# guzba/zippy

Hardware: AMD Instinct MI355X
Metric: GiB/s uncompressed throughput (compress BestSpeed + uncompress), 4096x1 MiB batch (higher is better)
Workload: dtype u8

## Files before the change

### zippy_amd/csrc/zh_l1_match.hip

```cpp
#include <cstdlib>
#include <cstring>

#include "zh_common.h"
#include "zh_kprof.h"
#include "zh_tables.h"

namespace {
constexpr uint32_t kHashMul = 0x1e35a7bdu;
constexpr uint32_t kCntWords = 1024;
constexpr uint32_t kBitsWords = 512, kFlagBits = 12, kFlagWords = (1u << kFlagBits) / 32u;
static_assert(kBitsWords + 2u * kFlagWords <= kCntWords, "the parse's maps lie inside the coverage bitmap's words");
constexpr uint32_t kHistWords = ZH_HIST_STRIDE / 2;
static_assert(ZH_HIST_STRIDE % 2 == 0, "packed pairs");
struct __attribute__((packed)) Bytes16 {
  uint32_t x, y, z, w;
};

}

template <bool kLdsTable>
__global__ __launch_bounds__(64) void zh_l1_match_kernel(const uint8_t* __restrict__ d_src,
                                                         ZhCompressArgs a, int huffman_only,
                                                         uint16_t* __restrict__ table_pool,
                                                         uint32_t* __restrict__ next_frag,
                                                         const uint32_t* __restrict__ order,
                                                         uint32_t* __restrict__ cost, uint32_t ticket_base) {
  __shared__ uint32_t s_hist[kHistWords];
  __shared__ uint32_t s_scr[kCntWords];
  __shared__ uint32_t s_nmatch;
  uint32_t* const s_bits = s_scr;
  uint32_t* const s_seen = s_scr + kBitsWords;
  uint32_t* const s_dup = s_seen + kFlagWords;
  uint32_t* const s_cover = s_scr;

  const unsigned lane = zh_lane();
  __shared__ uint16_t s_table_lds[kLdsTable ? 16384 : 2];
  uint16_t* const s_table = kLdsTable ? s_table_lds : table_pool + (size_t)blockIdx.x * 16384u;
  uint32_t taken = 0;
  for (uint32_t ticket = ticket_base + blockIdx.x; ticket < a.nfrags; taken++) {
  const uint32_t f = order ? order[ticket] : ticket;
  const uint64_t t_start = zh_clock();
  KPROF_DECL(16);
  const ZhFragDesc fd = a.frags[f];
  const uint32_t n = fd.len;
  const uint8_t* src = d_src + fd.src_off;
  uint16_t* m_pos = a.m_pos + (size_t)f * ZH_MAX_MATCHES_PER_FRAG;
  uint16_t* m_len = a.m_len + (size_t)f * ZH_MAX_MATCHES_PER_FRAG;
  uint16_t* m_off = a.m_off + (size_t)f * ZH_MAX_MATCHES_PER_FRAG;

  const uint32_t mis = (uint32_t)((uintptr_t)src & 3u);
  const uint32_t* asrc = reinterpret_cast<const uint32_t*>(src - mis);
  const uint32_t last_dw = n ? (n + mis - 1u) >> 2 : 0u;
  auto dw = [&](uint32_t i) -> uint32_t { return asrc[i < last_dw ? i : last_dw]; };
  auto ld32 = [&](uint32_t p) -> uint32_t {
    const uint32_t q = p + mis, i = q >> 2;
    return __builtin_amdgcn_alignbyte(dw(i + 1), dw(i), q);
  };
  uint32_t table_size = 256, shift = 24;
  while (table_size < 16384u && table_size < n) {
    table_size <<= 1;
    shift--;
  }
  const uint32_t e0 = (!huffman_only && n >= 4) ? (((ld32(0) * kHashMul) >> 17) & 1u) << 15 : 0u;
  for (uint32_t i = lane; i < kBitsWords + 2u * kFlagWords; i += 64) s_scr[i] = 0;
  zh_wave_sync();
  KPROF_MARK(0);

  {
    uint32_t nm = 0;
    if (!huffman_only && n >= 15) {
      const uint32_t ip_limit = n - 15;
      uint32_t ip = 1;
      uint32_t K = 0;
      bool post = false;
      bool finished = false;
      while (!finished) {
        const bool dense = post || K < 32u;
        uint32_t pos, step, W0 = 0;
        if (dense) {
          W0 = post ? ip - 1u : ip;
          pos = W0 + lane;
          step = 1;
        } else {
          const uint32_t s = 32 + K, q = s >> 5, r = s & 31u, j = lane;
          uint32_t off = q * j;
          if (j > 32u - r) off += j - (32u - r);
          if (j > 64u - r) off += j - (64u - r);
          pos = ip + off;
          step = (s + j) >> 5;
        }
        const bool valid = pos + step <= ip_limit;
        if (!valid) pos = 1;
        Bytes16 av = {0, 0, 0, 0};
        if (valid) av = *reinterpret_cast<const Bytes16*>(src + pos);
        const uint32_t a0 = av.x, a1 = av.y, a2 = av.z, a3 = av.w;
        const uint32_t hp = a0 * kHashMul;
        const uint32_t h = hp >> shift, tag = (hp >> 17) & 1u;
        uint32_t oldw = e0;
        if (valid && ((s_bits[h >> 5] >> (h & 31u)) & 1u))
          oldw = kLdsTable ? (uint32_t)s_table[h]
                           : (uint32_t)__hip_atomic_load(s_table + h, __ATOMIC_RELAXED, __HIP_MEMORY_SCOPE_AGENT);
        const uint32_t old = oldw & 0x7fffu;
        const bool fetch = valid && (oldw >> 15) == tag;
        const uint32_t ck = (h & ((1u << kFlagBits) - 1u)) >> 5, cb = 1u << (h & 31u);
        const uint32_t seen_before = valid ? atomicOr(&s_seen[ck], cb) : 0u;
        Bytes16 qv = {0, 0, 0, 0};
        if (fetch) qv = *reinterpret_cast<const Bytes16*>(src + old);
        if (seen_before & cb) atomicOr(&s_dup[ck], cb);
        zh_wave_sync();
        const bool flagged = valid && (s_dup[ck] & cb);
        zh_wave_sync();
        if (valid) s_seen[ck] = s_dup[ck] = 0;
        const uint32_t x0 = fetch ? a0 ^ qv.x : 1u;
        const uint32_t x1 = a1 ^ qv.y;
        const uint32_t x2 = a2 ^ qv.z;
        const uint32_t x3 = a3 ^ qv.w;
        const uint32_t c0 = min(((uint32_t)__ffs((int)x0) - 1u) >> 3, 4u);
        const uint32_t c1 = min(((uint32_t)__ffs((int)x1) - 1u) >> 3, 4u);
        const uint32_t c2 = min(((uint32_t)__ffs((int)x2) - 1u) >> 3, 4u);
        const uint32_t c3 = min(((uint32_t)__ffs((int)x3) - 1u) >> 3, 4u);
        const uint32_t c23 = c2 + (c2 == 4u ? c3 : 0u);
        const uint32_t c123 = c1 + (c1 == 4u ? c23 : 0u);
        const uint32_t eqlen = c0 + (c0 == 4u ? c123 : 0u);

        const uint64_t V = __ballot(valid);
        const uint64_t H = __ballot(valid && x0 == 0);
        const uint64_t C = __ballot(flagged);
        uint64_t Cw = C;
        if (C && __popcll(C) <= 16) {
          Cw = 0;
          for (uint64_t cm = C; cm; cm &= cm - 1) {
            const uint32_t g = (uint32_t)__ffsll((long long)cm) - 1u;
            const uint32_t hg = __builtin_amdgcn_readlane(h, g);
            const bool same_h = valid && h == hg;
            if (__ballot(same_h) & ((1ull << g) - 1ull)) Cw |= 1ull << g;
          }
        }
        const uint32_t t = V == ~0ull ? 64u : (uint32_t)__ffsll((long long)~V) - 1u;

        KPROF_MARK(1);
        KPROF_COUNT(6, 1);
#ifndef ZH_EMU
        __builtin_amdgcn_s_setprio(1);
#endif
        uint64_t ins = post ? 1ull : 0ull;
        uint32_t i = post ? 1u : 0u;
        bool reprobe = post;
        uint32_t hop = 0x8000u;
        if (dense) {
          const uint64_t ev = (H | Cw) >> lane;
          const uint32_t d = ev ? (uint32_t)__ffsll((long long)ev) - 1u : 64u;
          const uint32_t info = eqlen | ((uint32_t)((Cw >> lane) & 1ull) << 5);
          const uint32_t gi = (uint32_t)__shfl((int)info, (int)((lane + d) & 63u), 64);
          if (d < 32u && gi < 16u) {
            const uint32_t g0 = lane + d, nx = g0 + gi;
            hop = g0 | 0x40u | (nx << 8) | ((d + 1u) << 16) | ((nx <= 64u ? nx - 1u : g0) << 22);
          } else if (!ev && lane >= 32u) {
            hop = 63u | (64u << 8);
          }
        }
        const uint32_t tt = ip_limit > W0 ? ip_limit - W0 : 0u;
        for (;;) {
          if (dense && i < 64u) {
            uint64_t sel = 0;
            uint32_t cur = zh_bcast(i), tv = 0x8000u;
            KPROF_MARK(3);
            bool go = true;
            if (!reprobe && K) {
              tv = __builtin_amdgcn_readlane(hop, cur);
              go = !(tv & 0x8000u) && (tv & 0x40u) && K + ((tv & 63u) - cur) <= 31u;
            }
            const uint32_t lim = zh_bcast(tt < 64u ? tt : 64u);
            if (go && cur < lim) {
#ifdef ZH_EMU
              do {
                tv = __builtin_amdgcn_readlane(hop, cur);
                if ((tv & 0x8040u) != 0x40u) break;
                const uint32_t g = tv & 63u, nxt = (tv >> 8) & 127u;
                sel |= 1ull << g;
                ins |= (~0ull << cur) & (~0ull >> (63u - g));
                ins |= 1ull << (nxt <= 64u ? nxt - 1u : g);
                cur = nxt;
              } while (cur < lim);
#else
              uint32_t t0, g, nxt;
              uint64_t m1;
              asm volatile(
                  "1:\n\t"
                  "v_readlane_b32 %[tv], %[hop], %[cur]\n\t"
                  "s_bitcmp1_b32 %[tv], 6\n\t"
                  "s_cbranch_scc0 2f\n\t"
                  "s_and_b32 %[g], %[tv], 63\n\t"
                  "s_bitset1_b64 %[sel], %[g]\n\t"
                  "s_bfe_u32 %[t0], %[tv], 0x60010\n\t"
                  "s_bfm_b64 %[m1], %[t0], %[cur]\n\t"
                  "s_or_b64 %[ins], %[ins], %[m1]\n\t"
                  "s_bfe_u32 %[t0], %[tv], 0x60016\n\t"
                  "s_bitset1_b64 %[ins], %[t0]\n\t"
                  "s_bfe_u32 %[cur], %[tv], 0x70008\n\t"
                  "s_cmp_lt_u32 %[cur], %[lim]\n\t"
                  "s_cbranch_scc1 1b\n\t"
                  "2:"
                  : [tv] "=&s"(tv), [cur] "+s"(cur), [sel] "+s"(sel), [ins] "+s"(ins), [t0] "=&s"(t0),
                    [g] "=&s"(g), [nxt] "=&s"(nxt), [m1] "=&s"(m1)
                  : [hop] "v"(hop), [lim] "s"(lim)
                  : "scc");
#endif
            }
            const bool chained = cur != i;
            bool run_out = false;
            if (go && cur < lim && !(tv & 0x8040u) && tt >= 64u) {
              K = (chained || reprobe ? 63u : K + 64u) - cur;
              ins |= ~0ull << cur;
              run_out = true;
            }
            KPROF_MARK(2);
            if (sel) {
              KPROF_COUNT(8, __popcll(sel));
              if ((sel >> lane) & 1ull) {
                const uint32_t k = nm + (uint32_t)__popcll(sel & zh_lanemask_lt());
                zh_store_nt(m_pos + k, (uint16_t)pos);
                zh_store_nt(m_len + k, (uint16_t)eqlen);
                zh_store_nt(m_off + k, (uint16_t)(pos - old));
              }
              nm += (uint32_t)__popcll(sel);
            }
            if (run_out) {
              post = false;
              ip = W0 + 64u;
              break;
            }
            if (chained) {
              K = 0;
              if (cur >= tt) {
                finished = true;
                break;
              }
              if (cur >= 64u) {
                post = true;
                ip = W0 + cur;
                break;
              }
              i = cur;
              reprobe = true;
            }
          }
          KPROF_COUNT(9, 1);
          if (i >= t) {
            finished = true;
            break;
          }
          uint32_t g = i;
          if (!reprobe) {
            const uint32_t last_dense = dense ? i + (31u - K) : 63u;
            uint32_t lim = last_dense < 63u ? last_dense : 63u;
            if (t - 1u < lim) lim = t - 1u;
            const uint64_t E = (H | Cw) & (~0ull << i);
            g = E ? (uint32_t)__ffsll((long long)E) - 1u : 64u;
            if (g > lim) {
              KPROF_COUNT(12, 1);
              ins |= (~0ull << i) & (~0ull >> (63u - lim));
              if (dense && lim == last_dense) {
                K = 32;
                ip = W0 + lim + 1u;
                post = false;
              } else if (lim + 1u == t && t < 64u) {
                finished = true;
              } else {
                K += 64u - i;
                post = false;
                if (dense) {
                  ip = W0 + 64u;
                } else {
                  ip = __builtin_amdgcn_readlane(pos, 63) + __builtin_amdgcn_readlane(step, 63);
                }
              }
              break;
            }
            if (g > i) ins |= (~0ull << i) & ((1ull << g) - 1ull);
            K += g - i;
          }
          uint32_t cand, flen;
          bool hit;
          if ((Cw >> g) & 1ull) {
            KPROF_COUNT(14, 1);
            const uint32_t hg = __builtin_amdgcn_readlane(h, g);
            const uint64_t same = __ballot(h == hg) & ins;
            if (same) {
              const uint32_t k = 63u - (uint32_t)__clzll((long long)same);
              cand = __builtin_amdgcn_readlane(pos, k);
              hit = __builtin_amdgcn_readlane(a0, k) == __builtin_amdgcn_readlane(a0, g);
              flen = 4;
              if (hit) {
                const uint32_t y1 = (uint32_t)__builtin_amdgcn_readlane(a1, k) ^ (uint32_t)__builtin_amdgcn_readlane(a1, g);
                if (y1) {
                  flen = 4u + (((uint32_t)__ffs((int)y1) - 1u) >> 3);
                } else {
                  const uint32_t y2 = (uint32_t)__builtin_amdgcn_readlane(a2, k) ^ (uint32_t)__builtin_amdgcn_readlane(a2, g);
                  if (y2) {
                    flen = 8u + (((uint32_t)__ffs((int)y2) - 1u) >> 3);
                  } else {
                    const uint32_t y3 = (uint32_t)__builtin_amdgcn_readlane(a3, k) ^ (uint32_t)__builtin_amdgcn_readlane(a3, g);
                    flen = y3 ? 12u + (((uint32_t)__ffs((int)y3) - 1u) >> 3) : 16u;
                  }
                }
              }
            } else {
              cand = __builtin_amdgcn_readlane(old, g);
              hit = (H >> g) & 1ull;
              flen = __builtin_amdgcn_readlane(eqlen, g);
            }
          } else {
            cand = __builtin_amdgcn_readlane(old, g);
            hit = (H >> g) & 1ull;
            flen = __builtin_amdgcn_readlane(eqlen, g);
          }
          ins |= 1ull << g;
          if (!hit) {
            if (reprobe) {
              reprobe = false;
              K = 0;
            } else {
              K++;
            }
            i = g + 1u;
            if (dense && K == 32u) {
              ip = W0 + i;
              post = false;
              break;
            }
            if (i >= 64u) {
              post = false;
              ip = dense ? W0 + 64u
                         : __builtin_amdgcn_readlane(pos, 63) + __builtin_amdgcn_readlane(step, 63);
              break;
            }
            continue;
          }
          const uint32_t mp = __builtin_amdgcn_readlane(pos, g);
          const uint32_t limit = n < mp + 258u ? n : mp + 258u;
          uint32_t matched;
          if (flen < 16u) {
            KPROF_COUNT(15, 1);
            matched = flen;
          } else {
            KPROF_COUNT(10, 1);
            zh_wave_sync();
            const uint32_t o = flen + 4u * lane;
            uint32_t avail = 0;
            if (mp + o < limit) avail = limit - (mp + o) < 4u ? limit - (mp + o) : 4u;
            const uint32_t x = ld32(mp + o) ^ ld32(cand + o);
            uint32_t eq = min(((uint32_t)__ffs((int)x) - 1u) >> 3, 4u);
            if (eq > avail) eq = avail;
            const uint64_t stop = __ballot(eq < 4u);
            const uint32_t fl = (uint32_t)__ffsll((long long)stop) - 1u;
            matched = flen + 4u * fl + __builtin_amdgcn_readlane(eq, fl);
          }
          if (matched > limit - mp) matched = limit - mp;
          if (lane == 0) {
            zh_store_nt(m_pos + nm, (uint16_t)mp);
            zh_store_nt(m_len + nm, (uint16_t)matched);
            zh_store_nt(m_off + nm, (uint16_t)(mp - cand));
          }
          nm++;
          ip = mp + matched;
          K = 0;
          post = true;
          if (ip >= ip_limit) {
            finished = true;
            break;
          }
          const uint32_t ni = g + matched;
          if (!dense || ni >= 64u) break;
          ins |= 1ull << (ni - 1u);
          i = ni;
          reprobe = true;
        }
        KPROF_MARK(3);
#ifndef ZH_EMU
        __builtin_amdgcn_s_setprio(0);
#endif
        if (finished) break;
        const bool mine = (ins >> lane) & 1ull;
        if (mine) atomicOr(&s_bits[h >> 5], 1u << (h & 31u));
        if (mine && !((C >> lane) & 1ull)) s_table[h] = (uint16_t)(pos | (tag << 15));
        uint64_t cc = ins & C;
        while (cc) {
          const uint32_t jx = (uint32_t)__ffsll((long long)cc) - 1u;
          cc &= cc - 1;
          if (lane == jx) s_table[h] = (uint16_t)(pos | (tag << 15));
        }
        zh_wave_sync();
        KPROF_MARK(4);
      }
    }
    if (lane == 0) s_nmatch = nm;
  }
  __threadfence_block();
  zh_wave_sync();
  KPROF_MARK(3);
  const uint32_t nmatch = s_nmatch;
  for (uint32_t i = lane; i < kCntWords; i += 64) s_scr[i] = 0;
  for (uint32_t i = lane; i < kHistWords; i += 64) s_hist[i] = 0;
  zh_wave_sync();

  uint32_t extra_bits = 0, covered = 0;
  auto hist_add = [&](uint32_t sym) { atomicAdd(&s_hist[sym >> 1], 1u << (16u * (sym & 1u))); };
  {
    const uint32_t mlast = nmatch ? nmatch - 1u : 0u;
    auto at = [&](uint32_t m) { return m < nmatch ? m : mlast; };
    uint32_t pq = m_pos[at(lane)], lq = m_len[at(lane)], oq = m_off[at(lane)];
    for (uint32_t m = lane; m - lane < nmatch; m += 64) {
      const uint32_t p = pq, l = lq, o = oq;
      pq = m_pos[at(m + 64u)];
      lq = m_len[at(m + 64u)];
      oq = m_off[at(m + 64u)];
      if (m < nmatch) {
        const uint32_t li = zh_len_code(l), di = zh_dist_code(o);
        hist_add(257u + li);
        hist_add(ZH_NUM_LITLEN + di);
        extra_bits += zh_len_extra_bits(li) + zh_dist_extra_bits(di);
        covered += l;
        atomicXor(&s_cover[(p + 1u) >> 5], 1u << ((p + 1u) & 31u));
        if (p + l < kCntWords * 32u) atomicXor(&s_cover[(p + l) >> 5], 1u << ((p + l) & 31u));
      }
    }
  }
  zh_wave_sync();
  {
    uint32_t carry = 0;
    for (uint32_t w0 = 0; w0 < kCntWords && w0 * 32u < n; w0 += 64) {
      uint32_t x = s_cover[w0 + lane];
#pragma unroll
      for (uint32_t sh = 1; sh < 32; sh <<= 1) x ^= x << sh;
      const uint64_t odd = __ballot((x >> 31) != 0u);
      if ((carry + (uint32_t)__popcll(odd & zh_lanemask_lt())) & 1u) x = ~x;
      s_cover[w0 + lane] = x;
      carry += (uint32_t)__popcll(odd);
    }
  }
  zh_wave_sync();
  if (a.f_cover) {
    uint32_t* cov_out = a.f_cover + (size_t)f * kCntWords;
    for (uint32_t w0 = 0; w0 * 32u < n; w0 += 64) cov_out[w0 + lane] = s_cover[w0 + lane];
  }
  for (uint32_t base = 0; base < n; base += 1024) {
    uint32_t wq[4];
#pragma unroll
    for (uint32_t u = 0; u < 4; u++) {
      const uint32_t p = base + 256u * u + 4u * lane;
      wq[u] = p < n ? ld32(p) : 0u;
    }
#pragma unroll
    for (uint32_t u = 0; u < 4; u++) {
      const uint32_t p = base + 256u * u + 4u * lane;
      if (p < n) {
        const uint32_t wi = p >> 5;
        const uint32_t c_lo = s_cover[wi], c_hi = wi + 1u < kCntWords ? s_cover[wi + 1u] : 0u;
        const uint32_t cov = (uint32_t)((((uint64_t)c_hi << 32) | c_lo) >> (p & 31u));
        const uint32_t notlit = cov | (cov >> 1);
#pragma unroll
        for (uint32_t k = 0; k < 4; k++)
          if (p + k < n && !((notlit >> k) & 1u)) hist_add((wq[u] >> (8u * k)) & 255u);
      }
    }
  }
  extra_bits = zh_wave_sum(extra_bits);
  covered = zh_wave_sum(covered);
  zh_wave_sync();

  uint16_t* hist_out = a.f_hist + (size_t)f * ZH_HIST_STRIDE;
  for (uint32_t i = lane; i < ZH_HIST_STRIDE; i += 64) hist_out[i] = (uint16_t)(s_hist[i >> 1] >> (16u * (i & 1u)));
  if (lane == 0) {
    a.f_nmatch[f] = nmatch;
    a.f_spill[f] = 0;
    a.f_nlit[f] = n - covered;
    a.f_extra_bits[f] = extra_bits;
  }
  KPROF_MARK(5);
  KPROF_COUNT(11, 1);
  KPROF_FLUSH(0, 16);
  zh_wave_sync();
  {
    uint32_t nf = 0;
    if (lane == 0) {
      if (cost) {
        const uint64_t dt = zh_clock() - t_start;
        cost[f] = dt < 0xffffffffull ? (uint32_t)dt : 0xffffffffu;
      }
      nf = atomicAdd(next_frag, 1u);
    }
    ticket = zh_bcast(nf);
  }
  }
  if (lane == 0 && taken) atomicAdd(next_frag + (kLdsTable ? 2 : 1), taken);
}

namespace {
constexpr uint32_t kCostClasses = 64;
__device__ __forceinline__ uint32_t cost_class(uint32_t c) {
  if (c < 1024u) return 0u;
  const uint32_t lg = 31u - (uint32_t)__clz((int)c);
  const uint32_t k = (lg - 10u) * 4u + ((c >> (lg - 2u)) & 3u);
  return k < kCostClasses ? k : kCostClasses - 1u;
}
}
__global__ __launch_bounds__(256) void zh_l1_cost_hist_kernel(const uint32_t* __restrict__ cost, uint32_t n,
                                                              uint32_t* __restrict__ hist) {
  __shared__ uint32_t s_h[kCostClasses];
  if (threadIdx.x < kCostClasses) s_h[threadIdx.x] = 0;
  __syncthreads();
  const uint32_t i = blockIdx.x * 256u + threadIdx.x;
  if (i < n) atomicAdd(&s_h[cost_class(cost[i])], 1u);
  __syncthreads();
  if (threadIdx.x < kCostClasses && s_h[threadIdx.x]) atomicAdd(&hist[threadIdx.x], s_h[threadIdx.x]);
}
__global__ __launch_bounds__(64) void zh_l1_cost_places_kernel(uint32_t* __restrict__ hist) {
  const unsigned lane = zh_lane();
  const uint32_t mine = hist[kCostClasses - 1u - lane];
  const uint32_t incl = zh_wave_scan(mine);
  hist[kCostClasses + (kCostClasses - 1u - lane)] = incl - mine;
}
__global__ __launch_bounds__(256) void zh_l1_cost_sort_kernel(const uint32_t* __restrict__ cost, uint32_t n,
                                                              uint32_t* __restrict__ hist, uint32_t* __restrict__ order) {
  const uint32_t i = blockIdx.x * 256u + threadIdx.x;
  if (i < n) order[atomicAdd(&hist[kCostClasses + cost_class(cost[i])], 1u)] = i;
}
__global__ __launch_bounds__(64) void zh_l1_cost_cut_kernel(uint32_t* __restrict__ hist, uint32_t tail) {
  const unsigned lane = zh_lane();
  const uint32_t incl = zh_wave_scan(hist[lane]);
  const uint64_t fits = __ballot(incl <= tail);
  const uint32_t k = (uint32_t)__popcll(fits);
  if (lane == 0) hist[kCostClasses] = k ? k - 1u : 0xffffffffu;
  if (lane == (k ? k - 1u : 0u)) hist[kCostClasses + 1u] = k ? incl : 0u;
}
__global__ __launch_bounds__(256) void zh_l1_cost_count_kernel(const uint32_t* __restrict__ cost, uint32_t n,
                                                               const uint32_t* __restrict__ hist,
                                                               uint32_t* __restrict__ blk) {
  const uint32_t i = blockIdx.x * 256u + threadIdx.x, cut = hist[kCostClasses];
  const bool last = i < n && cut != 0xffffffffu && cost_class(cost[i]) <= cut;
  const uint32_t c = (uint32_t)__popcll(__ballot(last));
  __shared__ uint32_t s_c[4];
  if (zh_lane() == 0) s_c[threadIdx.x >> 6] = c;
  __syncthreads();
  if (threadIdx.x == 0) blk[blockIdx.x] = s_c[0] + s_c[1] + s_c[2] + s_c[3];
}
__global__ __launch_bounds__(1024) void zh_l1_cost_scan_kernel(uint32_t* __restrict__ blk, uint32_t nblk) {
  __shared__ uint32_t s_w[16], s_carry;
  const uint32_t tid = threadIdx.x;
  if (tid == 0) s_carry = 0;
  __syncthreads();
  for (uint32_t base = 0; base < nblk; base += 1024u) {
    const uint32_t i = base + tid, v = i < nblk ? blk[i] : 0u;
    const uint32_t incl = zh_wave_scan(v);
    if (zh_lane() == 63) s_w[tid >> 6] = incl;
    __syncthreads();
    uint32_t before = s_carry;
    for (uint32_t w = 0; w < (tid >> 6); w++) before += s_w[w];
    if (i < nblk) blk[i] = before + incl - v;
    __syncthreads();
    if (tid == 1023) s_carry = before + incl;
    __syncthreads();
  }
}
__global__ __launch_bounds__(256) void zh_l1_cost_scatter_kernel(const uint32_t* __restrict__ cost, uint32_t n,
                                                                 const uint32_t* __restrict__ hist,
                                                                 const uint32_t* __restrict__ blk,
                                                                 uint32_t* __restrict__ order) {
  const uint32_t i = blockIdx.x * 256u + threadIdx.x, cut = hist[kCostClasses], ntail = hist[kCostClasses + 1u];
  const bool last = i < n && cut != 0xffffffffu && cost_class(cost[i]) <= cut;
  const uint64_t m = __ballot(last);
  __shared__ uint32_t s_c[4];
  if (zh_lane() == 0) s_c[threadIdx.x >> 6] = (uint32_t)__popcll(m);
  __syncthreads();
  uint32_t before = blk[blockIdx.x] + (uint32_t)__popcll(m & zh_lanemask_lt());
  for (uint32_t w = 0; w < (threadIdx.x >> 6); w++) before += s_c[w];
  if (i < n) order[last ? (n - ntail) + before : i - before] = i;
}

namespace {
long l1_slots_env() {
  static const long v = [] {
    const char* e = getenv("ZH_L1_SLOTS");
    const long v = e ? atol(e) : 0;
    return v >= 1 && v <= 16384 ? v : 0;
  }();
  return v;
}
uint32_t l1_lds_waves() {
  static const uint32_t waves = [] {
    const char* e = getenv("ZH_L1_LDS_WAVES");
    const long v = e ? atol(e) : -1;
    return v >= 0 && v <= 1024 ? (uint32_t)v : 512u;
  }();
  return waves;
}
}

extern "C" uint32_t zh_l1_table_slots(void) { return l1_slots_env() ? (uint32_t)l1_slots_env() : 4864u; }

__global__ void zh_l1_set_counter_kernel(uint32_t* next_frag, uint32_t v) {
  next_frag[0] = v;
  next_frag[1] = next_frag[2] = 0;
}

__global__ void zh_l1_head_start_kernel() {}

extern "C" ZhL1Launch zh_l1_match_prepare(hipStream_t stream, uint32_t nfrags, uint32_t* next_frag, uint32_t* cost,
                                          uint32_t* order, uint32_t* hist, int use_order, int side_ok) {
  ZhL1Launch l = {0, 0, nullptr};
  if (!nfrags) return l;
#ifdef ZH_XCHECK
  static const bool lds = [] {
    const char* e = getenv("ZH_L1_TABLE");
    return e && strcmp(e, "lds") == 0;
  }();
  if (lds) {
    l.lds = nfrags < 1024u ? nfrags : 1024u;
    hipLaunchKernelGGL(zh_l1_set_counter_kernel, dim3(1), dim3(1), 0, stream, next_frag, l.lds);
    return l;
  }
#endif
  const uint32_t mixed_pooled = l1_slots_env() ? (uint32_t)l1_slots_env() : 4096u;
  if (side_ok && l1_lds_waves() && nfrags >= mixed_pooled + l1_lds_waves()) {
    l.pooled = mixed_pooled;
    l.lds = l1_lds_waves();
  } else {
    l.pooled = nfrags < zh_l1_table_slots() ? nfrags : zh_l1_table_slots();
  }
  const uint32_t grid = l.pooled + l.lds;
  const bool sorted = use_order && cost && order && hist && nfrags > grid;
  if (sorted) {
    const uint32_t g = (nfrags + 255u) / 256u;
    static const uint32_t rounds = [] {
      const char* e = getenv("ZH_L1_TAIL_ROUNDS");
      const long v = e ? atol(e) : 0;
      return v >= 1 && v <= 64 ? (uint32_t)v : 2u;
    }();
    const uint32_t tail = nfrags / 2u < rounds * grid ? nfrags / 2u : rounds * grid;
    uint32_t* blk = hist + 128;
    (void)hipMemsetAsync(hist, 0, 128u * sizeof(uint32_t), stream);
    hipLaunchKernelGGL(zh_l1_cost_hist_kernel, dim3(g), dim3(256), 0, stream, cost, nfrags, hist);
    if (nfrags < 8u * grid) {
      hipLaunchKernelGGL(zh_l1_cost_places_kernel, dim3(1), dim3(64), 0, stream, hist);
      hipLaunchKernelGGL(zh_l1_cost_sort_kernel, dim3(g), dim3(256), 0, stream, cost, nfrags, hist, order);
    } else {
      hipLaunchKernelGGL(zh_l1_cost_cut_kernel, dim3(1), dim3(64), 0, stream, hist, tail);
      hipLaunchKernelGGL(zh_l1_cost_count_kernel, dim3(g), dim3(256), 0, stream, cost, nfrags, hist, blk);
      hipLaunchKernelGGL(zh_l1_cost_scan_kernel, dim3(1), dim3(1024), 0, stream, blk, g);
      hipLaunchKernelGGL(zh_l1_cost_scatter_kernel, dim3(g), dim3(256), 0, stream, cost, nfrags, hist, blk, order);
    }
    l.order = order;
  }
  hipLaunchKernelGGL(zh_l1_set_counter_kernel, dim3(1), dim3(1), 0, stream, next_frag, grid);
  return l;
}

extern "C" void zh_launch_l1_match(hipStream_t stream, const uint8_t* d_src, ZhCompressArgs a, int huffman_only,
                                   uint16_t* table_pool, uint32_t* next_frag, uint32_t* cost, ZhL1Launch l,
                                   int lds_part) {
  if (lds_part) {
    if (l.lds)
      hipLaunchKernelGGL(zh_l1_match_kernel<true>, dim3(l.lds), dim3(64), 0, stream, d_src, a, huffman_only, table_pool,
                         next_frag, l.order, cost, l.pooled);
  } else if (l.pooled) {
    static const uint32_t head_start = [] {
      const char* e = getenv("ZH_L1_HEAD_START");
      const long v = e ? atol(e) : -1;
      return v >= 0 && v <= 16 ? (uint32_t)v : 3u;
    }();
    for (uint32_t i = 0; l.lds && i < head_start; i++)
      hipLaunchKernelGGL(zh_l1_head_start_kernel, dim3(1), dim3(1), 0, stream);
    hipLaunchKernelGGL(zh_l1_match_kernel<false>, dim3(l.pooled), dim3(64), 0, stream, d_src, a, huffman_only,
                       table_pool, next_frag, l.order, cost, 0u);
  }
}
```

Baseline: 48.82.

## Add lean pooled L1 match kernel with reduced LDS and rebalance LDS/pooled waves

Adds a lean variant of the pooled match kernel. It reuses the parse's bitmap region for the coverage map and histogram, and processes coverage in two partitions with a seam bit, cutting LDS use per wave. The LDS-table variant drops the occupancy bitmap, pre-fills the table with the sentinel entry instead, and packs the table and flag maps into one array. Defaults shift work toward more LDS-table waves (768) and fewer pooled slots (3840), aiming for higher occupancy and less global-table traffic. The cost is extra partition passes and a more complex coverage computation.

```diff
diff --git a/zippy_amd/csrc/zh_l1_match.hip b/zippy_amd/csrc/zh_l1_match.hip
--- a/zippy_amd/csrc/zh_l1_match.hip
+++ b/zippy_amd/csrc/zh_l1_match.hip
@@ -18,24 +18,31 @@
 
 }
 
-template <bool kLdsTable>
+template <bool kLdsTable, bool kLean>
 __global__ __launch_bounds__(64) void zh_l1_match_kernel(const uint8_t* __restrict__ d_src,
                                                          ZhCompressArgs a, int huffman_only,
                                                          uint16_t* __restrict__ table_pool,
                                                          uint32_t* __restrict__ next_frag,
                                                          const uint32_t* __restrict__ order,
                                                          uint32_t* __restrict__ cost, uint32_t ticket_base) {
-  __shared__ uint32_t s_hist[kHistWords];
-  __shared__ uint32_t s_scr[kCntWords];
+  constexpr bool kClassic = !kLdsTable && !kLean;
+  static_assert(!(kLdsTable && kLean), "the lean form is a pooled one");
+  constexpr uint32_t kParts = kLean ? 2u : 1u, kPartWords = kCntWords / kParts, kPartBits = kPartWords * 32u;
+  static_assert(kPartWords + kHistWords <= kBitsWords + 2u * kFlagWords || !kLean, "the lean statistics lie inside the parse's maps");
+  static_assert(kPartBits % 2048u == 0, "whole groups of 64 words, whole passes of the literal histogram");
+  __shared__ uint32_t s_hist_own[kClassic ? kHistWords : 1];
+  __shared__ uint32_t s_scr[kClassic ? kCntWords : 1];
   __shared__ uint32_t s_nmatch;
-  uint32_t* const s_bits = s_scr;
-  uint32_t* const s_seen = s_scr + kBitsWords;
+  __shared__ uint32_t s_lean[kLean ? kBitsWords + 2u * kFlagWords : 1];
+  __shared__ __attribute__((aligned(16))) uint32_t s_lds[kLdsTable ? 8192u + 2u * kFlagWords : 1];
+  uint32_t* const s_bits = kClassic ? s_scr : s_lean;
+  uint32_t* const s_seen = kLdsTable ? s_lds + 8192 : s_bits + kBitsWords;
   uint32_t* const s_dup = s_seen + kFlagWords;
-  uint32_t* const s_cover = s_scr;
+  uint32_t* const s_cover = kLdsTable ? s_lds : s_bits;
+  uint32_t* const s_hist = kClassic ? s_hist_own : s_cover + kPartWords;
 
   const unsigned lane = zh_lane();
-  __shared__ uint16_t s_table_lds[kLdsTable ? 16384 : 2];
-  uint16_t* const s_table = kLdsTable ? s_table_lds : table_pool + (size_t)blockIdx.x * 16384u;
+  uint16_t* const s_table = kLdsTable ? reinterpret_cast<uint16_t*>(s_lds) : table_pool + (size_t)blockIdx.x * 16384u;
   uint32_t taken = 0;
   for (uint32_t ticket = ticket_base + blockIdx.x; ticket < a.nfrags; taken++) {
   const uint32_t f = order ? order[ticket] : ticket;
@@ -62,10 +69,21 @@
     shift--;
   }
   const uint32_t e0 = (!huffman_only && n >= 4) ? (((ld32(0) * kHashMul) >> 17) & 1u) << 15 : 0u;
-  for (uint32_t i = lane; i < kBitsWords + 2u * kFlagWords; i += 64) s_scr[i] = 0;
+  if constexpr (kLdsTable) {
+    for (uint32_t i = lane; i < 2u * kFlagWords; i += 64) s_seen[i] = 0;
+    if (!huffman_only && n >= 15) {
+      const uint32_t e2 = e0 | (e0 << 16);
+      const uint4 fill = {e2, e2, e2, e2};
+      uint4* const t4 = reinterpret_cast<uint4*>(s_lds);
+      for (uint32_t i = lane; i < table_size / 8u; i += 64) t4[i] = fill;
+    }
+  } else {
+    for (uint32_t i = lane; i < kBitsWords + 2u * kFlagWords; i += 64) s_bits[i] = 0;
+  }
   zh_wave_sync();
   KPROF_MARK(0);
 
+  uint32_t nm_parse = 0;
   {
     uint32_t nm = 0;
     if (!huffman_only && n >= 15) {
@@ -97,9 +115,12 @@
         const uint32_t hp = a0 * kHashMul;
         const uint32_t h = hp >> shift, tag = (hp >> 17) & 1u;
         uint32_t oldw = e0;
-        if (valid && ((s_bits[h >> 5] >> (h & 31u)) & 1u))
-          oldw = kLdsTable ? (uint32_t)s_table[h]
-                           : (uint32_t)__hip_atomic_load(s_table + h, __ATOMIC_RELAXED, __HIP_MEMORY_SCOPE_AGENT);
+        if constexpr (kLdsTable) {
+          if (valid) oldw = s_table[h];
+        } else {
+          if (valid && ((s_bits[h >> 5] >> (h & 31u)) & 1u))
+            oldw = (uint32_t)__hip_atomic_load(s_table + h, __ATOMIC_RELAXED, __HIP_MEMORY_SCOPE_AGENT);
+        }
         const uint32_t old = oldw & 0x7fffu;
         const bool fetch = valid && (oldw >> 15) == tag;
         const uint32_t ck = (h & ((1u << kFlagBits) - 1u)) >> 5, cb = 1u << (h & 31u);
@@ -382,7 +403,9 @@
 #endif
         if (finished) break;
         const bool mine = (ins >> lane) & 1ull;
-        if (mine) atomicOr(&s_bits[h >> 5], 1u << (h & 31u));
+        if constexpr (!kLdsTable) {
+          if (mine) atomicOr(&s_bits[h >> 5], 1u << (h & 31u));
+        }
         if (mine && !((C >> lane) & 1ull)) s_table[h] = (uint16_t)(pos | (tag << 15));
         uint64_t cc = ins & C;
         while (cc) {
@@ -394,18 +417,23 @@
         KPROF_MARK(4);
       }
     }
-    if (lane == 0) s_nmatch = nm;
+    if constexpr (kClassic) {
+      if (lane == 0) s_nmatch = nm;
+    } else {
+      nm_parse = zh_bcast(nm);
+    }
   }
   __threadfence_block();
   zh_wave_sync();
   KPROF_MARK(3);
-  const uint32_t nmatch = s_nmatch;
-  for (uint32_t i = lane; i < kCntWords; i += 64) s_scr[i] = 0;
+  const uint32_t nmatch = kClassic ? s_nmatch : nm_parse;
+  uint32_t extra_bits = 0, covered = 0;
+  auto hist_add = [&](uint32_t sym) { atomicAdd(&s_hist[sym >> 1], 1u << (16u * (sym & 1u))); };
+  if constexpr (!kLean) {
+  for (uint32_t i = lane; i < kCntWords; i += 64) s_cover[i] = 0;
   for (uint32_t i = lane; i < kHistWords; i += 64) s_hist[i] = 0;
   zh_wave_sync();
 
-  uint32_t extra_bits = 0, covered = 0;
-  auto hist_add = [&](uint32_t sym) { atomicAdd(&s_hist[sym >> 1], 1u << (16u * (sym & 1u))); };
   {
     const uint32_t mlast = nmatch ? nmatch - 1u : 0u;
     auto at = [&](uint32_t m) { return m < nmatch ? m : mlast; };
@@ -465,6 +493,102 @@
       }
     }
   }
+  } else {
+  uint32_t carry = 0, m_from = nmatch;
+  for (uint32_t lo = 0; lo < kCntWords * 32u && (lo < n || !lo); lo += kPartBits) {
+    if (lo) zh_wave_sync();
+    for (uint32_t i = lane; i < kPartWords; i += 64) s_cover[i] = 0;
+    if (!lo)
+      for (uint32_t i = lane; i < kHistWords; i += 64) s_hist[i] = 0;
+    zh_wave_sync();
+    uint32_t seam = 0;
+    {
+      const uint32_t mlast = nmatch ? nmatch - 1u : 0u;
+      auto at = [&](uint32_t m) { return m < nmatch ? m : mlast; };
+      constexpr uint32_t kGroups = 4;
+      const uint32_t m0 = lo ? m_from : 0u;
+      uint32_t pq[kGroups], lq[kGroups], oq[kGroups];
+#pragma unroll
+      for (uint32_t u = 0; u < kGroups; u++) {
+        const uint32_t k = at(m0 + 64u * u + lane);
+        pq[u] = m_pos[k];
+        lq[u] = m_len[k];
+        oq[u] = m_off[k];
+      }
+      for (uint32_t mb = m0; mb < nmatch; mb += 64u * kGroups) {
+        uint32_t pc[kGroups], lc[kGroups], oc[kGroups];
+#pragma unroll
+        for (uint32_t u = 0; u < kGroups; u++) {
+          pc[u] = pq[u];
+          lc[u] = lq[u];
+          oc[u] = oq[u];
+          const uint32_t k = at(mb + 64u * (kGroups + u) + lane);
+          pq[u] = m_pos[k];
+          lq[u] = m_len[k];
+          oq[u] = m_off[k];
+        }
+        bool reaches = false;
+#pragma unroll
+        for (uint32_t u = 0; u < kGroups; u++) {
+          const uint32_t m = mb + 64u * u + lane, p = pc[u], l = lc[u], o = oc[u];
+          if (m < nmatch) {
+            if (!lo) {
+              const uint32_t li = zh_len_code(l), di = zh_dist_code(o);
+              hist_add(257u + li);
+              hist_add(ZH_NUM_LITLEN + di);
+              extra_bits += zh_len_extra_bits(li) + zh_dist_extra_bits(di);
+              covered += l;
+            }
+            const uint32_t b0 = p + 1u - lo, b1 = p + l - lo;
+            if (b0 < kPartBits) atomicXor(&s_cover[b0 >> 5], 1u << (b0 & 31u));
+            if (b1 < kPartBits) atomicXor(&s_cover[b1 >> 5], 1u << (b1 & 31u));
+            seam ^= (uint32_t)(b0 == kPartBits) ^ (uint32_t)(b1 == kPartBits);
+            reaches |= p + l >= lo + kPartBits;
+          }
+        }
+        if (!lo && m_from == nmatch && __ballot(reaches)) m_from = mb;
+      }
+    }
+    zh_wave_sync();
+    for (uint32_t w0 = 0; w0 < kPartWords && lo + w0 * 32u < n; w0 += 64) {
+      uint32_t x = s_cover[w0 + lane];
+#pragma unroll
+      for (uint32_t sh = 1; sh < 32; sh <<= 1) x ^= x << sh;
+      const uint64_t odd = __ballot((x >> 31) != 0u);
+      if ((carry + (uint32_t)__popcll(odd & zh_lanemask_lt())) & 1u) x = ~x;
+      s_cover[w0 + lane] = x;
+      carry += (uint32_t)__popcll(odd);
+    }
+    zh_wave_sync();
+    if (a.f_cover) {
+      uint32_t* cov_out = a.f_cover + (size_t)f * kCntWords + (lo >> 5);
+      for (uint32_t w0 = 0; w0 < kPartWords && lo + w0 * 32u < n; w0 += 64) cov_out[w0 + lane] = s_cover[w0 + lane];
+    }
+    const uint32_t seam_bit =
+        lo + kPartBits < kCntWords * 32u ? (carry + (uint32_t)__popcll(__ballot((seam & 1u) != 0u))) & 1u : 0u;
+    for (uint32_t base = lo; base < n && base < lo + kPartBits; base += 1024) {
+      uint32_t wq[4];
+#pragma unroll
+      for (uint32_t u = 0; u < 4; u++) {
+        const uint32_t p = base + 256u * u + 4u * lane;
+        wq[u] = p < n ? ld32(p) : 0u;
+      }
+#pragma unroll
+      for (uint32_t u = 0; u < 4; u++) {
+        const uint32_t p = base + 256u * u + 4u * lane;
+        if (p < n) {
+          const uint32_t wi = (p - lo) >> 5;
+          const uint32_t c_lo = s_cover[wi], c_hi = wi + 1u < kPartWords ? s_cover[wi + 1u] : seam_bit;
+          const uint32_t cov = (uint32_t)((((uint64_t)c_hi << 32) | c_lo) >> (p & 31u));
+          const uint32_t notlit = cov | (cov >> 1);
+#pragma unroll
+          for (uint32_t k = 0; k < 4; k++)
+            if (p + k < n && !((notlit >> k) & 1u)) hist_add((wq[u] >> (8u * k)) & 255u);
+        }
+      }
+    }
+  }
+  }
   extra_bits = zh_wave_sum(extra_bits);
   covered = zh_wave_sum(covered);
   zh_wave_sync();
@@ -591,7 +715,7 @@
   static const uint32_t waves = [] {
     const char* e = getenv("ZH_L1_LDS_WAVES");
     const long v = e ? atol(e) : -1;
-    return v >= 0 && v <= 1024 ? (uint32_t)v : 512u;
+    return v >= 0 && v <= 1024 ? (uint32_t)v : 768u;
   }();
   return waves;
 }
@@ -621,7 +745,7 @@
     return l;
   }
 #endif
-  const uint32_t mixed_pooled = l1_slots_env() ? (uint32_t)l1_slots_env() : 4096u;
+  const uint32_t mixed_pooled = l1_slots_env() ? (uint32_t)l1_slots_env() : 3840u;
   if (side_ok && l1_lds_waves() && nfrags >= mixed_pooled + l1_lds_waves()) {
     l.pooled = mixed_pooled;
     l.lds = l1_lds_waves();
@@ -661,7 +785,7 @@
                                    int lds_part) {
   if (lds_part) {
     if (l.lds)
-      hipLaunchKernelGGL(zh_l1_match_kernel<true>, dim3(l.lds), dim3(64), 0, stream, d_src, a, huffman_only, table_pool,
+      hipLaunchKernelGGL((zh_l1_match_kernel<true, false>), dim3(l.lds), dim3(64), 0, stream, d_src, a, huffman_only, table_pool,
                          next_frag, l.order, cost, l.pooled);
   } else if (l.pooled) {
     static const uint32_t head_start = [] {
@@ -671,7 +795,15 @@
     }();
     for (uint32_t i = 0; l.lds && i < head_start; i++)
       hipLaunchKernelGGL(zh_l1_head_start_kernel, dim3(1), dim3(1), 0, stream);
-    hipLaunchKernelGGL(zh_l1_match_kernel<false>, dim3(l.pooled), dim3(64), 0, stream, d_src, a, huffman_only,
-                       table_pool, next_frag, l.order, cost, 0u);
-  }
-}
+    static const bool lean = [] {
+      const char* e = getenv("ZH_L1_LEAN");
+      return !(e && strcmp(e, "0") == 0);
+    }();
+    if (l.lds && lean)
+      hipLaunchKernelGGL((zh_l1_match_kernel<false, true>), dim3(l.pooled), dim3(64), 0, stream, d_src, a, huffman_only,
+                         table_pool, next_frag, l.order, cost, 0u);
+    else
+      hipLaunchKernelGGL((zh_l1_match_kernel<false, false>), dim3(l.pooled), dim3(64), 0, stream, d_src, a,
+                         huffman_only, table_pool, next_frag, l.order, cost, 0u);
+  }
+}
```

Result: no change. 48.62 (-0.4%).
